# lucanest/Phyloformer

Hardware: AMD Instinct MI355X
Metric: alignments/sec, 60-leaf/500-site LG+GC-like MSAs, Phyloformer forward (pf.ckpt) (higher is better)
Workload: dtype f16x3-split MFMA (two fp16 limbs per operand, 3 passes), fp32 accumulate/residual

## Files before the change

### include/phyloformer_amd.h

```cpp
#ifndef PHYLOFORMER_AMD_H
#define PHYLOFORMER_AMD_H

#include <stddef.h>
#include <stdint.h>

#ifdef __cplusplus
extern "C" {
#endif

#define PF_ABI_VERSION 5

typedef enum pf_status {
    PF_OK = 0,
    PF_EINVAL = -1,
    PF_EHIP = -2,
    PF_ERCCL = -3,
    PF_ENOMEM = -4,
    PF_ESTATE = -5,
    PF_EIO = -6
} pf_status;

typedef struct pf_weights_t {
    int32_t n_blocks;
    int32_t n_heads;
// ... 46 lines not shown

int pf_forward_sharded(pf_handle_t* h, const uint8_t* idx, int32_t B, int32_t N,
                       int32_t l_begin, int32_t l_end, int32_t L_total, float* out);
int pf_forward_sharded_device(pf_handle_t* h, const uint8_t* d_idx, int32_t B, int32_t N,
                              int32_t l_begin, int32_t l_end, int32_t L_total, float* d_out);

#define PF_UNIQUE_ID_BYTES 256
int pf_comm_unique_id(void* id_out);
int pf_comm_init(pf_handle_t* h, const void* unique_id, int32_t rank, int32_t world_size);
int pf_comm_destroy(pf_handle_t* h);
int pf_comm_info(char* path_out, size_t path_cap, int32_t* version);

int pf_synchronize(pf_handle_t* h);
int pf_get_stream(pf_handle_t* h, void** hip_stream_out);
int pf_device_malloc(pf_handle_t* h, size_t bytes, void** out);
int pf_device_free(pf_handle_t* h, void* p);
int pf_memcpy_h2d(pf_handle_t* h, void* dst, const void* src, size_t bytes);
int pf_memcpy_d2h(pf_handle_t* h, void* dst, const void* src, size_t bytes);

int pf_profile_reset(pf_handle_t* h);
int pf_profile_get(pf_handle_t* h, const char* kernel, int64_t* launches, double* total_ms);

int64_t pf_debug_read(pf_handle_t* h, const char* name, float* dst, int64_t cap);

int pf_device_info(pf_handle_t* h, char* name_out, size_t name_cap, int32_t* cu_count,
                   uint64_t* hbm_bytes);
int pf_device_pci(pf_handle_t* h, int32_t* domain, int32_t* bus, int32_t* device);

int pf_forward_shards_emulated(pf_handle_t* h, const uint8_t* idx, int32_t B, int32_t N, int32_t L,
                               int32_t nshards, float* out);

int pf_selftest(pf_handle_t* h, float* out);

typedef struct pf_mha_weights_t {
    int32_t n_heads;
    int32_t embed_dim;
    const float *wq, *bq, *wk, *bk, *wv, *bv, *wo, *bo;
} pf_mha_weights_t;
typedef struct pf_mha pf_mha_t;
int pf_create_bare(int device, pf_handle_t** out);
int pf_mha_create(pf_handle_t* h, const pf_mha_weights_t* w, pf_mha_t** out);
int pf_mha_destroy(pf_mha_t* m);
int pf_mha_forward(pf_mha_t* m, const float* x, int32_t B, int32_t R, int32_t C, float* y);
int pf_mha_forward_device(pf_mha_t* m, const float* d_x, int32_t B, int32_t R, int32_t C, float* d_y);

#define PF_FASTA_EBYTE (-16)
#define PF_FASTA_ERAGGED (-17)
#define PF_FASTA_ENOHEADER (-18)
#define PF_FASTA_EEMPTY (-19)
#define PF_FASTA_ECAP (-20)
#define PF_FASTA_EUTF8 (-21)
int pf_parse_fasta(const char* data, int64_t len, uint8_t* idx, int64_t idx_cap, int64_t* id_spans,
                   int32_t max_seqs, int32_t* n_out, int32_t* l_out, int64_t* detail);

int64_t pf_format_phylip(const float* preds, int32_t n, const char* const* ids, char* out, int64_t cap);
int64_t pf_format_phylip_n(const float* preds, int32_t n, const char* const* ids, const int64_t* id_lens, char* out,
                           int64_t cap);

int64_t pf_nj_newick_n(const float* preds, int32_t n, const char* const* ids, const int64_t* id_lens, int32_t clamp_negative,
                       char* out, int64_t cap);

typedef struct pf_fasta_batch pf_fasta_batch_t;
int pf_fasta_batch_load(const char* const* paths, int32_t count, int32_t threads, pf_fasta_batch_t** out);
void pf_fasta_batch_free(pf_fasta_batch_t* b);
int32_t pf_fasta_batch_count(const pf_fasta_batch_t* b);
int pf_fasta_batch_infos(const pf_fasta_batch_t* b, int32_t* status, int32_t* n, int32_t* l, int64_t* detail);
// ... 12 lines not shown
```

### phyloformer_amd/csrc/pf_device.hip.h

```cpp
#pragma once
#include <hip/hip_runtime.h>
#include <stdint.h>

#include "pf_layout.h"

namespace pfk {

typedef float f32x4 __attribute__((ext_vector_type(4)));
typedef float f32x16 __attribute__((ext_vector_type(16)));
#if PF_F16
typedef _Float16 h16_t;
#define PF_MFMA(a, b, c) __builtin_amdgcn_mfma_f32_32x32x16_f16((a), (b), (c), 0, 0, 0)
#define PF_DOT2C "v_dot2c_f32_f16"
#define PF_CVT_PK "v_cvt_pk_f16_f32"
#define PF_NEG1_LO 0x0000bc00u
#define PF_NEG1_HI 0xbc000000u
#else
typedef __bf16 h16_t;
#define PF_MFMA(a, b, c) __builtin_amdgcn_mfma_f32_32x32x16_bf16((a), (b), (c), 0, 0, 0)
#define PF_DOT2C "v_dot2c_f32_bf16"
#define PF_CVT_PK "v_cvt_pk_bf16_f32"
#define PF_NEG1_LO 0x0000bf80u
#define PF_NEG1_HI 0xbf800000u
#endif
// ... 242 lines not shown
        xn[j] = x[j] - mean;
        v4[j & 3] = fmaf(xn[j], xn[j], v4[j & 3]);
    }
    const float v = (v4[0] + v4[1]) + (v4[2] + v4[3]);
    const float rstd = __builtin_amdgcn_rsqf(pair_sum(v) * (1.f / 64.f) + LN_EPS);
#pragma unroll
    for (int j = 0; j < 32; ++j) xn[j] *= rstd;
}

typedef const f32x4 __attribute__((address_space(3)))* lds_f32x4_t;
__device__ __forceinline__ void load_acc_bias(f32x16& acc, lds_f32_t lds_bias_h) {
#pragma unroll
    for (int q4 = 0; q4 < 4; ++q4) {
        const f32x4 bb = *(lds_f32x4_t)(lds_bias_h + 8 * q4);
#pragma unroll
        for (int i = 0; i < 4; ++i) acc[4 * q4 + i] = bb[i];
    }
}

__device__ __forceinline__ void load_acc_bias(f32x16& acc, const float* lds_bias, int h) {
#pragma unroll
    for (int q4 = 0; q4 < 4; ++q4) {
        const f32x4 bb = *reinterpret_cast<const f32x4*>(lds_bias + 8 * q4 + 4 * h);
#pragma unroll
        for (int i = 0; i < 4; ++i) acc[4 * q4 + i] = bb[i];
    }
}

__device__ __forceinline__ frag_t zero_frag() {
    frag_t z;
#pragma unroll
    for (int i = 0; i < 8; ++i) z[i] = (h16_t)0.f;
    return z;
}

#ifndef PF_DEVICE_HELPERS_ONLY
struct MainArgs {
    float* x;
    float* qrow;
    const float* qcol;
    const frag_t* mfrag;
    const float* rq;
    const float* ctx;
    float* spart;
    float* outpart;
    const frag_t* wimg;
    const float* consts;
    const frag_t* wv_lo;
    const float* table;
    const uint8_t* idx;
    const int16_t* pair_i;
    const int16_t* pair_j;
    int B, N, P, Lloc;
    int flat;
    int nt_aln;
    int slots_aln;
    size_t trash_tok;
    int store_x_last;
    unsigned long long* prof;
    int ablate;
    float* sitemap;
};

enum { MODE_FIRST = 0, MODE_MID = 1, MODE_LAST = 2, MODE_MID0 = 3, MODE_LAST_FOLD = 4 };

struct TilePos { int b, kt, r0, l0; };
// ... 52 lines not shown
    constexpr bool FOLD = MODE == MODE_LAST_FOLD;
    static_assert(!SITEMAP || LAST, "the site map is the head's: last block only");
    extern __shared__ __attribute__((aligned(16))) unsigned char smem[];
    lds_frag_t lw = (lds_frag_t)smem;
    lds_f32_t lc = (lds_f32_t)(smem + FRAG_END * 16);

    {
        const float cv = a.consts[min((int)threadIdx.x, CONST_LEN - 1)];
        if (FOLD) {
            image_to_lds<FRAG_W1, FRAG_W2>(a.wimg, smem);
            image_to_lds<FRAG_WO, FRAG_U + U_FRAGS>(a.wimg, smem);
        } else {
            image_to_lds<(MODE == MODE_FIRST) ? FRAG_WV : 0, LAST ? FRAG_WV : FRAG_END>(a.wimg, smem);
        }
        static_assert(CONST_LEN <= MAIN_THREADS, "one constant per thread");
        if (threadIdx.x < CONST_LEN) reinterpret_cast<float*>(smem + FRAG_END * 16)[threadIdx.x] = cv;
        asm volatile("s_waitcnt vmcnt(0)" ::: "memory");
    }
    __syncthreads();

    const int lane = threadIdx.x & 63;
    const int wave = __builtin_amdgcn_readfirstlane(threadIdx.x >> 6);
    const int t = lane & 31;
    const int h = lane >> 5;
    const int ntiles = (a.Lloc + 31) >> 5;
    const int ntasks = a.B * a.nt_aln;
    if (wave >= MAIN_WAVES / 2) __builtin_amdgcn_s_setprio(1);
    unsigned long long tacc[6] = {0, 0, 0, 0, 0, 0}, tprev = 0;
#define PF_TICK(k) do { if (a.prof) { const unsigned long long tn_ = __builtin_amdgcn_s_memtime(); tacc[k] += tn_ - tprev; tprev = tn_; } } while (0)
    if (a.prof) tprev = __builtin_amdgcn_s_memtime();
    lds_frag_t w1p = lw + FRAG_W1 + lane;
    lds_frag_t w2p = lw + FRAG_W2 + lane;
    lds_frag_t wop = lw + FRAG_WO + lane;
    lds_frag_t qkp = lw + FRAG_QK + h * 8 + (t & 7);
    lds_f32_t lch = lc + 4 * h;
    PF_OPAQUE(wop); PF_OPAQUE(qkp); PF_OPAQUE(lch);
    lds_frag_t wvp = wop + (FRAG_WV - FRAG_WO);
    lds_f32_t luh = (lds_f32_t)(smem + FRAG_U * 16) + 16 * h;

    {
        const int nwaves = gridDim.x * MAIN_WAVES;
#ifndef PF_RUN_MAX
#define PF_RUN_MAX 8
#endif
        const int run = max(1, min(PF_RUN_MAX, ntasks / (nwaves * 8)));
        int run0 = (blockIdx.x * MAIN_WAVES + wave) * run;
        const int task0 = run0, task1 = ntasks;
        TilePos cur = tile_pos<FLAT>(a, min(task0, ntasks - 1), ntiles);
        int frag_row = -1;
        frag_t mfr[4];
        f32x4 rqv = {0.f, 0.f, 0.f, 0.f};
        f32x4 px[8], pctx[8], pqr, pqc;
        int pri = 0, prj = 0;
        auto prefetch = [&](const TilePos& np) {
            const LanePos nl = lane_pos<FLAT>(a, np, t);
            const int ll = nl.l, pb = np.b;
            const size_t tk = nl.tok0 + nl.toff;
            if (MODE == MODE_MID0) {
                const uint8_t* ib = a.idx + (size_t)pb * a.N * a.Lloc + ll;
                const int pp = np.r0 + (nl.in_r1 ? 1 : 0);
                pri = residue(ib[(size_t)a.pair_i[pp] * a.Lloc]);
                prj = residue(ib[(size_t)a.pair_j[pp] * a.Lloc]);
            } else {
                const f32x4* xp = reinterpret_cast<const f32x4*>(a.x + tk * 64 + 4 * h);
#pragma unroll
                for (int g = 0; g < 8; ++g) px[g] = xp[2 * g];
            }
            pqr = *reinterpret_cast<const f32x4*>(a.qrow + tk * 4);
            pqc = *reinterpret_cast<const f32x4*>(a.qcol + tk * 4);
            if (MODE != MODE_FIRST) {
                int hq = h;
                asm volatile("" : "+v"(hq));
                const f32x4* cp = reinterpret_cast<const f32x4*>(a.ctx + ((size_t)pb * a.Lloc + ll) * 64 + 4 * hq);
#pragma unroll
                for (int g = 0; g < 8; ++g) pctx[g] = cp[2 * g];
            }
        };
        if (MODE != MODE_FIRST && task0 < task1) prefetch(cur);

        for (int task = task0; task < task1;) {
            const int b = cur.b;
            const int row = b * a.P + cur.r0;
            int ntask = task + 1;
            TilePos nxt = tile_next<FLAT>(a, cur);
            if (ntask == run0 + run) {
                run0 += nwaves * run;
                ntask = run0;
                if (ntask < task1) nxt = tile_pos<FLAT>(a, ntask, ntiles);
            }
            const LanePos lp = lane_pos<FLAT>(a, cur, t);
            const bool straddle = lp.wrap < 32;
            int ai = 0, aj = 0;
            if (MODE == MODE_FIRST) { const int pp = cur.r0 + (lp.in_r1 ? 1 : 0); ai = a.pair_i[pp]; aj = a.pair_j[pp]; }
            auto load_mfr = [&](int r) {
                const frag_t* mf = a.mfrag + (size_t)r * 128 + t;
#pragma unroll
                for (int q = 0; q < 4; ++q) mfr[q] = mf[q * 32];
                typedef const f32x4 __attribute__((address_space(4)))* const_f32x4_t;
                rqv = *(const_f32x4_t)(unsigned long long)(a.rq + (size_t)__builtin_amdgcn_readfirstlane(r) * 4);
                frag_row = r;
            };
            if (MODE != MODE_FIRST && row != frag_row) load_mfr(row);
            const bool valid = lp.valid;
            const int lc_ = lp.l;
            const size_t tok = lp.tok0 + lp.toff;
            float x[32];
            float zh[4] = {0.f, 0.f, 0.f, 0.f};

            if (MODE == MODE_FIRST) {
                const int ri = residue(a.idx[((size_t)b * a.N + ai) * a.Lloc + lc_]);
                const int rj = residue(a.idx[((size_t)b * a.N + aj) * a.Lloc + lc_]);
                const f32x4* ti = reinterpret_cast<const f32x4*>(a.table + ri * 64 + 4 * h);
                const f32x4* tj = reinterpret_cast<const f32x4*>(a.table + rj * 64 + 4 * h);
#pragma unroll
                for (int g = 0; g < 8; ++g) {
                    f32x4 u = ti[2 * g], w = tj[2 * g];
#pragma unroll
                    for (int i = 0; i < 4; ++i) x[4 * g + i] = u[i] + w[i];
                }
            } else {
                if (MODE == MODE_MID0) {
                    const f32x4* ti = reinterpret_cast<const f32x4*>(a.table + pri * 64 + 4 * h);
                    const f32x4* tj = reinterpret_cast<const f32x4*>(a.table + prj * 64 + 4 * h);
#pragma unroll
                    for (int g = 0; g < 8; ++g) {
                        const f32x4 u = ti[2 * g], w = tj[2 * g];
#pragma unroll
                        for (int i = 0; i < 4; ++i) x[4 * g + i] = u[i] + w[i];
                    }
                } else {
#pragma unroll
                    for (int g = 0; g < 8; ++g)
#pragma unroll
                        for (int i = 0; i < 4; ++i) x[4 * g + i] = px[g][i];
                }
                PF_TICK(0);
                if (!(a.ablate & 8)) {
                    f32x16 ya[2];
#pragma unroll
                    for (int j = 0; j < 32; ++j) ya[j >> 4][j & 15] = x[j];
                    {
                        const f32x4 qr = pqr;
                        auto mix = [&](const bool mine) {
                            float v[8];
#pragma unroll
                            for (int i = 0; i < 4; ++i) v[i] = mine ? qr[i] * rqv[i] : 0.f;
                            v[4] = v[5] = mine ? 1.f : 0.f;
                            v[6] = v[7] = 0.f;
                            frag_t qb_hi, qb_lo;
                            split8(v, qb_hi, qb_lo);
#pragma unroll
                            for (int To = 0; To < 2; ++To) mfma3(ya[To], mfr[To * 2], mfr[To * 2 + 1], qb_hi, qb_lo, To == 1);
                        };
                        mix(h == 0 && !lp.in_r1);
                        if (straddle) {
                            load_mfr(row + 1);
                            mix(h == 0 && lp.in_r1);
                        }
                    }
                    {
                        const f32x4 qc = pqc * COLAPPLY_B_SCALE;
                        float o[32];
#pragma unroll
                        for (int g = 0; g < 8; ++g) {
                            const f32x4 u = pctx[g];
#pragma unroll
                            for (int i = 0; i < 4; ++i) o[4 * g + i] = u[i] * qc[g >> 1];
                        }
#pragma unroll
                        for (int s = 0; s < 4; ++s) {
                            frag_t ob_hi, ob_lo;
                            split8(&o[8 * s], ob_hi, ob_lo);
#pragma unroll
                            for (int To = 0; To < 2; ++To) {
                                lds_frag_t f = wop + ((To * 4 + s) * 2) * 64;
                                const frag_t a_hi = f[0], a_lo = f[64];
                                mfma3(ya[To], a_hi, a_lo, ob_hi, ob_lo, To == 1);
                            }
                        }
                    }
#pragma unroll
                    for (int j = 0; j < 32; ++j) x[j] = ya[j >> 4][j & 15];
                }

                PF_TICK(1);
                if (FOLD) {
#pragma unroll
                    for (int g = 0; g < 8; ++g) {
                        const f32x4 w4 = *(lds_f32x4_t)(lch + CONST_HW + 8 * g);
#pragma unroll
// ... 80 lines not shown
                            }
                            mfma3(oa[To], fh, fl, g_hi[u], g_lo[u], To == 1);
                            fh = nh; fl = nl;
                        }
                    }
                    PF_TICK(3);
#pragma unroll
                    for (int j = 0; j < 32; ++j) x[j] = oa[j >> 4][j & 15];
                }
            }

            if (!LAST && !(a.ablate & 4)) {
                frag_t wl[8];
#pragma unroll
                for (int i = WVLO_LDS; i < 8; ++i) wl[i] = a.wv_lo[i * 64 + lane];
                __builtin_amdgcn_sched_barrier(0);
                {
                    const size_t stok = valid ? tok : a.trash_tok + t;
                    f32x4* xo = reinterpret_cast<f32x4*>(a.x + stok * 64 + 4 * h);
#pragma unroll
                    for (int g = 0; g < 8; ++g) {
                        f32x4 u = {x[4 * g], x[4 * g + 1], x[4 * g + 2], x[4 * g + 3]};
                        xo[2 * g] = u;
                    }
                }
                if (a.ablate & 32) { cur = nxt; task = ntask; continue; }
                f32x16 va[3];
                {
                    float xn[32];
                    ln_pair(x, xn);
                    frag_t xb_hi[4], xb_lo[4];
#pragma unroll
                    for (int s = 0; s < 4; ++s) split8(&xn[8 * s], xb_hi[s], xb_lo[s]);
#pragma unroll
                    for (int s = 0; s < 4; ++s) {
                        const frag_t q_hi = qkp[(s * 2) * 16], q_lo = qkp[(s * 2 + 1) * 16];
                        if (s == 0) mfma3_zero(va[2], q_hi, q_lo, xb_hi[s], xb_lo[s]);
                        else mfma3(va[2], q_hi, q_lo, xb_hi[s], xb_lo[s]);
                    }
#pragma unroll
                    for (int s = 0; s < 4; ++s)
#pragma unroll
                        for (int T = 0; T < 2; ++T) {
                            const frag_t f_hi = wvp[(T * 4 + s) * 64];
                            const frag_t f_lo = T * 4 + s < WVLO_LDS ? wvp[(FRAG_WVLO - FRAG_WV) + (T * 4 + s) * 64] : wl[T * 4 + s];
                            if (s == 0) mfma3_zero(va[T], f_hi, f_lo, xb_hi[s], xb_lo[s], T == 1);
                            else mfma3(va[T], f_hi, f_lo, xb_hi[s], xb_lo[s], T == 1);
                        }
                }
#pragma unroll
                for (int r = 0; r < 4; ++r) va[2][r] += lc[CONST_BQK + 4 * h + r];
                float qk[4], ot[4];
#pragma unroll
                for (int i = 0; i < 4; ++i) qk[i] = elu1_fast(va[2][i]);
#pragma unroll
                for (int i = 0; i < 4; ++i) ot[i] = pair_other(qk[i], h);
                float qn[4], kn[4];
#pragma unroll
                for (int i = 0; i < 4; ++i) {
                    qn[i] = h ? ot[i] : qk[i];
                    kn[i] = h ? qk[i] : ot[i];
                }
                {
                    const size_t stok = valid ? tok : a.trash_tok + t;
                    f32x4 qs = {qn[0], qn[1], qn[2], qn[3]};
                    *reinterpret_cast<f32x4*>(a.qrow + stok * 4) = qs;
                }
                const long slot0 = (long)b * a.slots_aln + cur.kt + (FLAT ? cur.r0 : 0);
                for (int part = 0; part < (straddle ? 2 : 1); ++part) {
                    float* sp = a.spart + (size_t)(slot0 + part) * SROW;
                    const float vm = (valid && lp.in_r1 == (part == 1)) ? 1.f : 0.f;
                    float km[4];
// ... 214 lines not shown
    }
    __syncthreads();
    if (ok) {
        const float* s = st[sub];
        const int hh = c >> 4;
        const float sk = s[68 + hh];
        ctx[sub][c] = (s[c] + bvc * sk) / sk;
        if (c < 4) {
            const float r = a.L_total / s[64 + c];
            rqs[sub][c] = r;
            a.rq[(size_t)pr * 4 + c] = r * a.b_scale;
        }
    }
    __syncthreads();
    if (ok) {
        float* m = a.mrow ? a.mrow + (size_t)pr * MROW : nullptr;
#pragma unroll
        for (int hh = 0; hh < 4; ++hh) {
            float acc = 0.f;
#pragma unroll
            for (int d = 0; d < 16; ++d) acc = fmaf(wo[hh][d], ctx[sub][16 * hh + d], acc);
            if (m) m[hh * 64 + c] = acc * rqs[sub][hh];
            mm[sub][hh][c] = acc * a.a_scale;
        }
        mm[sub][4][c] = biasc;
        mm[sub][5][c] = biascol;
    }
    __syncthreads();
    if (ok) {
        const int To = c >> 5, t = c & 31;
        float v[8];
#pragma unroll
        for (int i = 0; i < 8; ++i) v[i] = (i < 6) ? mm[sub][i][32 * To + t] : 0.f;
        frag_t hi, lo;
        split8(v, hi, lo);
        frag_t* mf = a.mfrag + (size_t)pr * MFRAG_PER_PAIR + To * 64 + t;
        mf[0] = hi;
        mf[32] = lo;
    }
    }
}

__global__ void k_rowsum(const float* spart, float* srow, int npairs, int nparts_, int flat, int P, int Lloc, int slots_aln) {
    const int i = blockIdx.x * blockDim.x + threadIdx.x;
    if (i >= npairs * SROW) return;
    const int pr = i / SROW, c = i - pr * SROW;
    long first;
    int nparts;
    part_range(flat, pr, nparts_, P, Lloc, slots_aln, &first, &nparts);
    const float* sp = spart + (size_t)first * SROW + c;
    float acc = 0.f;
    for (int k = 0; k < nparts; k += 8) {
        float v[8];
#pragma unroll
        for (int q = 0; q < 8; ++q) v[q] = k + q < nparts ? sp[(size_t)(k + q) * SROW] : 0.f;
#pragma unroll
        for (int q = 0; q < 8; ++q) acc += v[q];
    }
    srow[i] = acc;
}

__global__ void k_outsum(const float* outpart, float* out, int npairs, int nparts_, float inv_L_total, int flat, int P,
                         int Lloc, int slots_aln) {
    const int pr = blockIdx.x * blockDim.x + threadIdx.x;
    if (pr >= npairs) return;
    long first;
    int nparts;
    part_range(flat, pr, nparts_, P, Lloc, slots_aln, &first, &nparts);
    const float* sp = outpart + first;
    float acc = 0.f;
    for (int k = 0; k < nparts; k += 8) {
// ... 394 lines not shown

__global__ void k_accumulate(float* dst, const float* src, size_t n) {
    const size_t i = (size_t)blockIdx.x * blockDim.x + threadIdx.x;
    if (i < n) dst[i] += src[i];
}

__global__ void k_selftest(float* out) {
    const int lane = threadIdx.x;
    out[lane] = pair_sum((float)lane);
    out[64 + lane] = pair_other((float)lane, lane >> 5);
    out[128 + lane] = row16_sum((float)lane);
    out[192 + lane] = half32_sum((float)lane);
    frag_t A1, A2, Bf;
    const int m = lane & 31, kg = lane >> 5;
#pragma unroll
    for (int i = 0; i < 8; ++i) {
        const int k = 8 * kg + i;
        A1[i] = (h16_t)(float)(m + 32 * (k % 8));
        A2[i] = (h16_t)(float)k;
        Bf[i] = (h16_t)((k == (m & 15)) ? 1.f : 0.f);
    }
    f32x16 acc1, acc2;
#pragma unroll
    for (int r = 0; r < 16; ++r) { acc1[r] = 0.f; acc2[r] = 0.f; }
    acc1 = PF_MFMA(A1, Bf, acc1);
    acc2 = PF_MFMA(A2, Bf, acc2);
#pragma unroll
    for (int r = 0; r < 16; ++r) {
        out[256 + lane * 16 + r] = acc1[r];
        out[1280 + lane * 16 + r] = acc2[r];
    }
}

#endif

}
```

### phyloformer_amd/csrc/pf_host_prep.h

```cpp
#pragma once
#include <algorithm>
#include <cmath>
#include <cstdint>
#include <cstring>
#include <vector>

#include "pf_layout.h"

namespace pfhost {
using namespace pfk;

inline uint16_t f2bf(float f) {
    uint32_t u;
    std::memcpy(&u, &f, 4);
    if ((u & 0x7fffffffu) > 0x7f800000u) return uint16_t((u >> 16) | 0x40);
    u += 0x7fffu + ((u >> 16) & 1u);
    return uint16_t(u >> 16);
}
inline float bf2f(uint16_t b) {
    uint32_t u = uint32_t(b) << 16;
    float f;
    std::memcpy(&f, &u, 4);
    return f;
}
// ... 31 lines not shown
#if PF_F16
inline uint16_t f2x(float f) { return f2h(f); }
inline float x2f(uint16_t b) { return h2f(b); }
#else
inline uint16_t f2x(float f) { return f2bf(f); }
inline float x2f(uint16_t b) { return bf2f(b); }
#endif
inline int kmap_h(int j, int h) { return 8 * (j >> 2) + 4 * h + (j & 3); }

inline void pack_frags(const float* W, int M, int K, int Mpad, uint16_t* out, float scale = 1.f) {
    const int nT = Mpad / 32, nS = K / 16;
    for (int T = 0; T < nT; ++T)
        for (int s = 0; s < nS; ++s)
            for (int lane = 0; lane < 64; ++lane)
                for (int i = 0; i < 8; ++i) {
                    const int m = 32 * T + (lane & 31), k = kmap_h(8 * s + i, lane >> 5);
                    const float w = (m < M) ? W[(size_t)m * K + k] * scale : 0.f;
                    const uint16_t hi = f2x(w);
                    const uint16_t lo = f2x(w - x2f(hi));
                    const size_t base = ((size_t)(T * nS + s) * 2) * 64;
                    out[(base + lane) * 8 + i] = hi;
                    out[(base + 64 + lane) * 8 + i] = lo;
                }
}

inline void pack_qk_frags(const float* wq, const float* wk, uint16_t* qk) {
    for (int s = 0; s < 4; ++s)
        for (int kg = 0; kg < 2; ++kg)
            for (int m = 0; m < 8; ++m)
                for (int i = 0; i < 8; ++i) {
                    const int k = kmap_h(8 * s + i, kg);
                    const float w = (m < 4) ? wq[(size_t)m * E + k] : wk[(size_t)(m - 4) * E + k];
                    const uint16_t hi = f2x(w), lo = f2x(w - x2f(hi));
                    qk[(((size_t)s * 2 + 0) * 16 + kg * 8 + m) * 8 + i] = hi;
                    qk[(((size_t)s * 2 + 1) * 16 + kg * 8 + m) * 8 + i] = lo;
                }
}

inline void pack_row_stats(const float* wv, const float* wq, const float* wk, uint16_t* img_tail ,
                    uint16_t* wv_lo) {
    std::vector<uint16_t> full((size_t)2 * 4 * 2 * 64 * 8);
    pack_frags(wv, E, E, E, full.data());
    for (int T = 0; T < 2; ++T)
        for (int s = 0; s < 4; ++s)
            for (int lane = 0; lane < 64; ++lane)
                for (int i = 0; i < 8; ++i) {
                    const size_t src = (((size_t)(T * 4 + s) * 2) * 64 + lane) * 8 + i;
                    const size_t dst = ((size_t)(T * 4 + s) * 64 + lane) * 8 + i;
                    img_tail[dst] = full[src];
                    wv_lo[dst] = full[src + 64 * 8];
                }
    pack_qk_frags(wq, wk, img_tail + (size_t)(FRAG_QK - FRAG_WV) * 8);
}

inline void fold_head(const float* w2 , const float* b2, const float* hw, float hb, double w2_scale,
                      float* u_img , float* c0) {
    for (int T = 0; T < FF / 32; ++T)
        for (int h = 0; h < 2; ++h)
            for (int r = 0; r < 16; ++r) {
                const int k = 32 * T + kmap_h(r, h);
                double acc = 0.0;
                for (int c = 0; c < E; ++c) acc += (double)hw[c] * (double)w2[(size_t)c * FF + k];
                u_img[(T * 2 + h) * 16 + r] = (float)(acc * w2_scale);
            }
    double acc = (double)hb;
    for (int c = 0; c < E; ++c) acc += (double)hw[c] * (double)b2[c];
    *c0 = (float)acc;
}

// ... 132 lines not shown
```

### phyloformer_amd/csrc/pf_layout.h

```cpp
#pragma once

#ifndef PF_F16
#define PF_F16 1
#endif

namespace pfk {

constexpr int E = 64;
constexpr int NH = 4;
constexpr int HD = 16;
constexpr int FF = 256;
constexpr int NA = 22;
constexpr int SROW = 72;
constexpr int MROW = 4 * 64;
constexpr float LN_EPS = 1e-5f;

constexpr int FRAG_W1 = 0;
constexpr int FRAG_W2 = FRAG_W1 + 8 * 4 * 2 * 64;
constexpr int FRAG_WO = FRAG_W2 + 2 * 16 * 2 * 64;
constexpr int FRAG_WV = FRAG_WO + 2 * 4 * 2 * 64;
constexpr int FRAG_QK = FRAG_WV + 2 * 4 * 64;
#ifndef PF_WVLO_LDS
#define PF_WVLO_LDS 4
#endif
constexpr int WVLO_LDS = PF_WVLO_LDS;
constexpr int FRAG_WVLO = FRAG_QK + 4 * 2 * 16;
constexpr int FRAG_END = FRAG_WVLO + WVLO_LDS * 64;
constexpr int FRAG_U = FRAG_WV;
constexpr int U_FRAGS = FF * 4 / 16;
static_assert(FRAG_U + U_FRAGS <= FRAG_END, "the folded head fits the last block's tail");
constexpr int WVLO_FRAGS = 2 * 4 * 64;
constexpr int CONST_B1 = 0, CONST_B2 = 256, CONST_BQK = 320, CONST_HW = 328, CONST_HB = 392,
              CONST_C0 = 393, CONST_BOC = 400;
constexpr int CONST_LEN = 464;
constexpr int MAIN_LDS_BYTES = FRAG_END * 16 + CONST_LEN * 4;
constexpr int MFRAG_PER_PAIR = 2 * 2 * 32;

constexpr int MAIN_THREADS = 512;
constexpr int MAIN_WAVES = MAIN_THREADS / 64;

constexpr int PAIRTAB_ROWS = 22 * 22, PAIRTAB_W = 72;

}
```

### phyloformer_amd/csrc/pf_lib.hip

```cpp
#include <hip/hip_runtime.h>
#include <dlfcn.h>

#include <algorithm>
#include <cmath>
#include <cstdarg>
#include <cstdio>
#include <cstdlib>
#include <cstring>
#include <functional>
#include <map>
#include <mutex>
#include <string>
#include <vector>

#include "../../include/phyloformer_amd.h"
#include "pf_device.hip.h"
#include "pf_mha.hip.h"
#include "pf_precise.hip.h"
#include "pf_generic.hip.h"
#include "pf_boot.hip.h"
#include "pf_sites.hip.h"
#include "pf_sitemap.hip.h"
#include "pf_sites_host.h"
#include "pf_host_prep.h"
// ... 1701 lines not shown
    float* total = (float*)stage.alloc((size_t)B * P * SROW * sizeof(float));
    if (!total) return fail(h, PF_ENOMEM, "shard sum buffer");
    auto reduce = [&](bool site_sums) -> int {
        const size_t count = (size_t)B * P * (site_sums ? 1 : SROW);
        for (ShardRun& r : runs)
            if (!site_sums && (rc = launch_rowsum(h, r, &r.rs))) return rc;
        hipMemsetAsync(total, 0, count * sizeof(float), h->stream);
        for (ShardRun& r : runs) {
            hipLaunchKernelGGL(k_accumulate, dim3((unsigned)((count + 255) / 256)), dim3(256), 0, h->stream,
                               total, site_sums ? r.d_out : r.w.srow, count);
            r.rs = RowStats{total, 1, 0};
        }
        return PF_OK;
    };
    rc = schedule(h, runs.data(), runs.size(), reduce);
    if (!rc && (hipMemcpyAsync(out, total, (size_t)B * P * sizeof(float), hipMemcpyDeviceToHost, h->stream) != hipSuccess ||
                hipStreamSynchronize(h->stream) != hipSuccess))
        rc = fail(h, PF_EHIP, "result copy failed");
    return rc;
}

int pf_selftest(pf_handle_t* h, float* out) {
    if (!h || !out) return PF_EINVAL;
    float* d = nullptr;
    HIPCHK(h, hipMalloc((void**)&d, 2304 * sizeof(float)));
    hipLaunchKernelGGL(k_selftest, dim3(1), dim3(64), 0, h->stream, d);
    HIPCHK(h, hipGetLastError());
    HIPCHK(h, hipMemcpyAsync(out, d, 2304 * sizeof(float), hipMemcpyDeviceToHost, h->stream));
    HIPCHK(h, hipStreamSynchronize(h->stream));
    hipFree(d);
    return PF_OK;
}

struct pf_mha {
    pf_handle* h = nullptr;
    float* wfrag = nullptr;
    float* bias = nullptr;
    char* ws = nullptr;
    size_t ws_bytes = 0;
    float* d_x = nullptr;
    float* d_y = nullptr;
    size_t d_xy_bytes = 0;
};

int pf_mha_create(pf_handle_t* h, const pf_mha_weights_t* w, pf_mha_t** out) {
    if (!h || !w || !out) return PF_EINVAL;
    if (w->n_heads != MHA_H || w->embed_dim != E)
        return fail(h, PF_EINVAL, "softmax attention kernels are specialised for embed_dim 64 / 4 heads, got %d / %d",
                    w->embed_dim, w->n_heads);
    const float* ws[4] = {w->wq, w->wk, w->wv, w->wo};
    const float* bs[4] = {w->bq, w->bk, w->bv, w->bo};
    std::vector<uint16_t> img((size_t)MHA_WTOTAL * 8);
    std::vector<float> bias(4 * E);
    for (int i = 0; i < 4; ++i) {
        if (!ws[i] || !bs[i]) return fail(h, PF_EINVAL, "pf_mha_create: NULL weight pointer");
        std::copy(bs[i], bs[i] + E, bias.begin() + i * E);
    }
    pack_frags(w->wq, E, E, E, img.data());
    pack_frags(w->wk, E, E, E, img.data() + (size_t)MHA_OFF_WK * 8);
    pack_frags(w->wv, E, E, E, img.data() + (size_t)MHA_OFF_WV * 8);
    pack_frags(w->wo, E, E, E, img.data() + (size_t)MHA_OFF_WO * 8);
    HIPCHK(h, hipSetDevice(h->device));
    pf_mha* m = new pf_mha();
    m->h = h;
    void* p = nullptr;
    if (hipMalloc(&p, img.size() * 2) != hipSuccess) { delete m; return fail(h, PF_ENOMEM, "pf_mha_create: hipMalloc failed"); }
// ... 101 lines not shown
```

### phyloformer_amd/engine.py

```python
from __future__ import annotations

import ctypes as C
import os
from typing import Dict, Optional, Tuple

import numpy as np

from .weights import ModelWeights

HERE = os.path.dirname(os.path.abspath(__file__))
LIB_PATH = os.path.join(HERE, "libphyloformer_amd.so")
ABI_VERSION = 5
UNIQUE_ID_BYTES = 256

PF_OK, PF_EINVAL, PF_EHIP, PF_ERCCL, PF_ENOMEM, PF_ESTATE = 0, -1, -2, -3, -4, -5


def _refuse_single_sequence(B: int, N: int):
    if N == 1 and B >= 1:
        raise RuntimeError(f"cannot reshape tensor of 0 elements into shape [{B}, -1, 0, 64] because the unspecified "
                           "dimension size -1 can be any value and is ambiguous")


class EngineError(RuntimeError):
# ... 21 lines not shown
    "pf_forward_device": (C.c_int, [_H, C.c_void_p, C.c_int32, C.c_int32, C.c_int32, C.c_void_p]),
    "pf_resample_sites_device": (C.c_int, [_H, C.c_void_p, C.c_int32, C.c_int32, C.c_int32, C.c_int32, C.c_int32,
                                           C.c_uint64, C.c_void_p]),
    "pf_bootstrap": (C.c_int, [_H, C.c_void_p, C.c_int32, C.c_int32, C.c_int32, C.c_int32, C.c_uint64, C.c_void_p]),
    "pf_window_count": (C.c_int, [C.c_int32, C.c_int32, C.c_int32]),
    "pf_window_start": (C.c_int, [C.c_int32, C.c_int32, C.c_int32, C.c_int32]),
    "pf_gather_sites_device": (C.c_int, [_H, C.c_void_p, C.c_int32, C.c_int32, C.c_int32, C.c_void_p, C.c_void_p,
                                         C.c_int32, C.c_int32, C.c_void_p]),
    "pf_forward_sites": (C.c_int, [_H, C.c_void_p, C.c_int32, C.c_int32, C.c_int32, C.c_void_p, C.c_int32, C.c_int32,
                                   C.c_void_p]),
    "pf_forward_windows": (C.c_int, [_H, C.c_void_p, C.c_int32, C.c_int32, C.c_int32, C.c_int32, C.c_int32, C.c_void_p,
                                     C.c_int32]),
    "pf_forward_sharded": (C.c_int, [_H, C.c_void_p, C.c_int32, C.c_int32, C.c_int32, C.c_int32,
                                     C.c_int32, C.c_void_p]),
    "pf_forward_sharded_device": (C.c_int, [_H, C.c_void_p, C.c_int32, C.c_int32, C.c_int32,
                                            C.c_int32, C.c_int32, C.c_void_p]),
    "pf_comm_unique_id": (C.c_int, [C.c_void_p]),
    "pf_comm_init": (C.c_int, [_H, C.c_void_p, C.c_int32, C.c_int32]),
    "pf_comm_destroy": (C.c_int, [_H]),
    "pf_comm_info": (C.c_int, [C.c_char_p, C.c_size_t, C.POINTER(C.c_int32)]),
    "pf_synchronize": (C.c_int, [_H]),
    "pf_get_stream": (C.c_int, [_H, C.POINTER(C.c_void_p)]),
    "pf_device_malloc": (C.c_int, [_H, C.c_size_t, C.POINTER(C.c_void_p)]),
    "pf_device_free": (C.c_int, [_H, C.c_void_p]),
    "pf_memcpy_h2d": (C.c_int, [_H, C.c_void_p, C.c_void_p, C.c_size_t]),
    "pf_memcpy_d2h": (C.c_int, [_H, C.c_void_p, C.c_void_p, C.c_size_t]),
    "pf_profile_reset": (C.c_int, [_H]),
    "pf_profile_get": (C.c_int, [_H, C.c_char_p, C.POINTER(C.c_int64), C.POINTER(C.c_double)]),
    "pf_debug_read": (C.c_int64, [_H, C.c_char_p, C.c_void_p, C.c_int64]),
    "pf_device_info": (C.c_int, [_H, C.c_char_p, C.c_size_t, C.POINTER(C.c_int32),
                                 C.POINTER(C.c_uint64)]),
    "pf_device_pci": (C.c_int, [_H, C.POINTER(C.c_int32), C.POINTER(C.c_int32), C.POINTER(C.c_int32)]),
    "pf_selftest": (C.c_int, [_H, C.c_void_p]),
    "pf_create_bare": (C.c_int, [C.c_int, C.POINTER(_H)]),
    "pf_mha_create": (C.c_int, [_H, C.c_void_p, C.POINTER(C.c_void_p)]),
    "pf_mha_destroy": (C.c_int, [C.c_void_p]),
    "pf_mha_forward": (C.c_int, [C.c_void_p, C.c_void_p, C.c_int32, C.c_int32, C.c_int32, C.c_void_p]),
    "pf_mha_forward_device": (C.c_int, [C.c_void_p, C.c_void_p, C.c_int32, C.c_int32, C.c_int32, C.c_void_p]),
    "pf_parse_fasta": (C.c_int, [C.c_char_p, C.c_int64, C.c_void_p, C.c_int64, C.c_void_p, C.c_int32,
                                 C.POINTER(C.c_int32), C.POINTER(C.c_int32), C.POINTER(C.c_int64)]),
    "pf_format_phylip": (C.c_int64, [C.c_void_p, C.c_int32, C.POINTER(C.c_char_p), C.c_char_p, C.c_int64]),
    "pf_format_phylip_n": (C.c_int64, [C.c_void_p, C.c_int32, C.POINTER(C.c_char_p), C.c_void_p, C.c_char_p, C.c_int64]),
    "pf_fasta_batch_load": (C.c_int, [C.POINTER(C.c_char_p), C.c_int32, C.c_int32, C.POINTER(C.c_void_p)]),
    "pf_fasta_batch_free": (None, [C.c_void_p]),
    "pf_fasta_batch_count": (C.c_int32, [C.c_void_p]),
    "pf_fasta_batch_infos": (C.c_int, [C.c_void_p, C.c_void_p, C.c_void_p, C.c_void_p, C.c_void_p]),
    "pf_fasta_batch_id": (C.c_int, [C.c_void_p, C.c_int32, C.c_int32, C.POINTER(C.c_void_p), C.POINTER(C.c_int64)]),
    "pf_fasta_batch_gather": (C.c_int, [C.c_void_p, C.c_void_p, C.c_int32, C.c_int32, C.c_int32, C.c_void_p]),
    "pf_nj_newick_n": (C.c_int64, [C.c_void_p, C.c_int32, C.POINTER(C.c_char_p), C.c_void_p, C.c_int32, C.c_char_p, C.c_int64]),
    "pf_phylip_write_batch": (C.c_int, [C.c_void_p, C.c_void_p, C.c_int32, C.c_int32, C.c_void_p,
                                        C.POINTER(C.c_char_p), C.POINTER(C.c_char_p), C.c_int32, C.c_void_p]),
    "pf_forward_shards_emulated": (C.c_int, [_H, C.c_void_p, C.c_int32, C.c_int32, C.c_int32, C.c_int32,
                                             C.c_void_p]),
    "pf_forward_site_map": (C.c_int, [_H, C.c_void_p, C.c_int32, C.c_int32, C.c_int32, C.c_void_p, C.c_void_p]),
    "pf_forward_site_map_device": (C.c_int, [_H, C.c_void_p, C.c_int32, C.c_int32, C.c_int32, C.c_void_p, C.c_void_p]),
    "pf_forward_site_profile": (C.c_int, [_H, C.c_void_p, C.c_int32, C.c_int32, C.c_int32, C.c_void_p, C.c_void_p,
                                          C.c_void_p]),
    "pf_site_moments_device": (C.c_int, [_H, C.c_void_p, C.c_int32, C.c_int32, C.c_int32, C.c_void_p, C.c_void_p]),
}

CALL_TIME_SYMBOLS = frozenset({"pf_forward_site_map", "pf_forward_site_map_device", "pf_forward_site_profile",
                               "pf_site_moments_device"})

_lib: Optional[C.CDLL] = None


# ... 281 lines not shown
    def collective_count(self) -> int:
        return self.profile_get("collectives")[0]

    def rechecked_count(self) -> int:
        return self.profile_get("rechecked")[0]

    def comm_info(self) -> dict:
        buf = C.create_string_buffer(512)
        ver = C.c_int32()
        rc = self._lib.pf_comm_info(buf, 512, C.byref(ver))
        if rc != PF_OK:
            raise EngineError(rc, (self._lib.pf_last_error(None) or b"").decode())
        return {"library": buf.value.decode(), "version": int(ver.value)}

    def profile_reset(self):
        self._check(self._lib.pf_profile_reset(self._h))

    def profile_get(self, kernel: str) -> Tuple[int, float]:
        n = C.c_int64()
        ms = C.c_double()
        self._check(self._lib.pf_profile_get(self._h, kernel.encode(), C.byref(n), C.byref(ms)))
        return n.value, ms.value

    def debug_read(self, name: str) -> np.ndarray:
        n = self._check(self._lib.pf_debug_read(self._h, name.encode(), None, 0))
        out = np.empty(n, dtype=np.float32)
        self._check(self._lib.pf_debug_read(self._h, name.encode(), out.ctypes.data, n))
        return out

    def selftest(self) -> np.ndarray:
        out = np.empty(2304, dtype=np.float32)
        self._check(self._lib.pf_selftest(self._h, out.ctypes.data))
        return out
```

Measured before the change: 527.0.

## Stack hi/lo fp16 limbs into single MFMA K-dimension for mix and QK projections

New measurement: 531.8, median of 6. About the same (+0.9%).

```diff
diff --git a/include/phyloformer_amd.h b/include/phyloformer_amd.h
--- a/include/phyloformer_amd.h
+++ b/include/phyloformer_amd.h
@@ -102,6 +102,8 @@
 
 int pf_selftest(pf_handle_t* h, float* out);
 
+int pf_selftest_stacked(pf_handle_t* h, float* out);
+
 typedef struct pf_mha_weights_t {
     int32_t n_heads;
     int32_t embed_dim;
diff --git a/phyloformer_amd/csrc/pf_device.hip.h b/phyloformer_amd/csrc/pf_device.hip.h
--- a/phyloformer_amd/csrc/pf_device.hip.h
+++ b/phyloformer_amd/csrc/pf_device.hip.h
@@ -298,6 +298,26 @@
 #pragma unroll
     for (int i = 0; i < 8; ++i) z[i] = (h16_t)0.f;
     return z;
+}
+
+__device__ __forceinline__ void stack_mix_frags(const frag_t& hi, const frag_t& lo, frag_t& f0, frag_t& f1) {
+#pragma unroll
+    for (int i = 0; i < 6; ++i) f0[i] = hi[i];
+    f0[6] = lo[0]; f0[7] = lo[1];
+#pragma unroll
+    for (int i = 0; i < 4; ++i) { f1[i] = lo[2 + i]; f1[4 + i] = hi[i]; }
+}
+__device__ __forceinline__ frag_t mix_b_frag(unsigned qh0, unsigned ql0, unsigned qh1, unsigned ql1, unsigned one, int h) {
+    u32x4 b;
+    b[0] = h ? qh1 : qh0;
+    b[1] = h ? one : qh1;
+    b[2] = h ? ql0 : one;
+    b[3] = h ? ql1 : qh0;
+    return __builtin_bit_cast(frag_t, b);
+}
+__device__ __forceinline__ unsigned packed_ones() {
+    const h16x2 o = {(h16_t)1.f, (h16_t)1.f};
+    return __builtin_bit_cast(unsigned, o);
 }
 
 #ifndef PF_DEVICE_HELPERS_ONLY
@@ -416,7 +436,7 @@
     lds_frag_t w1p = lw + FRAG_W1 + lane;
     lds_frag_t w2p = lw + FRAG_W2 + lane;
     lds_frag_t wop = lw + FRAG_WO + lane;
-    lds_frag_t qkp = lw + FRAG_QK + h * 8 + (t & 7);
+    lds_frag_t qkp = lw + FRAG_QK + h * 16 + (t & 15);
     lds_f32_t lch = lc + 4 * h;
     PF_OPAQUE(wop); PF_OPAQUE(qkp); PF_OPAQUE(lch);
     lds_frag_t wvp = wop + (FRAG_WV - FRAG_WO);
@@ -432,7 +452,7 @@
         const int task0 = run0, task1 = ntasks;
         TilePos cur = tile_pos<FLAT>(a, min(task0, ntasks - 1), ntiles);
         int frag_row = -1;
-        frag_t mfr[4];
+        frag_t mfr[2];
         f32x4 rqv = {0.f, 0.f, 0.f, 0.f};
         f32x4 px[8], pctx[8], pqr, pqc;
         int pri = 0, prj = 0;
@@ -477,9 +497,9 @@
             int ai = 0, aj = 0;
             if (MODE == MODE_FIRST) { const int pp = cur.r0 + (lp.in_r1 ? 1 : 0); ai = a.pair_i[pp]; aj = a.pair_j[pp]; }
             auto load_mfr = [&](int r) {
-                const frag_t* mf = a.mfrag + (size_t)r * 128 + t;
-#pragma unroll
-                for (int q = 0; q < 4; ++q) mfr[q] = mf[q * 32];
+                const frag_t* mf = a.mfrag + (size_t)r * MFRAG_PER_PAIR + lane;
+#pragma unroll
+                for (int To = 0; To < 2; ++To) mfr[To] = mf[To * 64];
                 typedef const f32x4 __attribute__((address_space(4)))* const_f32x4_t;
                 rqv = *(const_f32x4_t)(unsigned long long)(a.rq + (size_t)__builtin_amdgcn_readfirstlane(r) * 4);
                 frag_row = r;
@@ -526,20 +546,20 @@
                     {
                         const f32x4 qr = pqr;
                         auto mix = [&](const bool mine) {
-                            float v[8];
+                            float v[4];
 #pragma unroll
                             for (int i = 0; i < 4; ++i) v[i] = mine ? qr[i] * rqv[i] : 0.f;
-                            v[4] = v[5] = mine ? 1.f : 0.f;
-                            v[6] = v[7] = 0.f;
-                            frag_t qb_hi, qb_lo;
-                            split8(v, qb_hi, qb_lo);
-#pragma unroll
-                            for (int To = 0; To < 2; ++To) mfma3(ya[To], mfr[To * 2], mfr[To * 2 + 1], qb_hi, qb_lo, To == 1);
+                            unsigned qh0, ql0, qh1, ql1;
+                            split_pair(v[0], v[1], qh0, ql0);
+                            split_pair(v[2], v[3], qh1, ql1);
+                            const frag_t qb = mix_b_frag(qh0, ql0, qh1, ql1, mine ? packed_ones() : 0u, h);
+#pragma unroll
+                            for (int To = 0; To < 2; ++To) ya[To] = PF_MFMA(mfr[To], qb, ya[To]);
                         };
-                        mix(h == 0 && !lp.in_r1);
+                        mix(!lp.in_r1);
                         if (straddle) {
                             load_mfr(row + 1);
-                            mix(h == 0 && lp.in_r1);
+                            mix(lp.in_r1);
                         }
                     }
                     {
@@ -686,12 +706,16 @@
                     frag_t xb_hi[4], xb_lo[4];
 #pragma unroll
                     for (int s = 0; s < 4; ++s) split8(&xn[8 * s], xb_hi[s], xb_lo[s]);
+                    f32x16 vl;
+                    const f32x16 z = {0.f, 0.f, 0.f, 0.f, 0.f, 0.f, 0.f, 0.f, 0.f, 0.f, 0.f, 0.f, 0.f, 0.f, 0.f, 0.f};
 #pragma unroll
                     for (int s = 0; s < 4; ++s) {
-                        const frag_t q_hi = qkp[(s * 2) * 16], q_lo = qkp[(s * 2 + 1) * 16];
-                        if (s == 0) mfma3_zero(va[2], q_hi, q_lo, xb_hi[s], xb_lo[s]);
-                        else mfma3(va[2], q_hi, q_lo, xb_hi[s], xb_lo[s]);
+                        const frag_t qf = qkp[s * 32];
+                        vl = PF_MFMA(qf, xb_lo[s], s == 0 ? z : vl);
+                        va[2] = PF_MFMA(qf, xb_hi[s], s == 0 ? z : va[2]);
                     }
+#pragma unroll
+                    for (int r = 0; r < 4; ++r) va[2][r] = (vl[r] + va[2][r]) + va[2][4 + r];
 #pragma unroll
                     for (int s = 0; s < 4; ++s)
 #pragma unroll
@@ -972,11 +996,12 @@
         float v[8];
 #pragma unroll
         for (int i = 0; i < 8; ++i) v[i] = (i < 6) ? mm[sub][i][32 * To + t] : 0.f;
-        frag_t hi, lo;
+        frag_t hi, lo, f0, f1;
         split8(v, hi, lo);
+        stack_mix_frags(hi, lo, f0, f1);
         frag_t* mf = a.mfrag + (size_t)pr * MFRAG_PER_PAIR + To * 64 + t;
-        mf[0] = hi;
-        mf[32] = lo;
+        mf[0] = f0;
+        mf[32] = f1;
     }
     }
 }
@@ -1437,6 +1462,46 @@
     }
 }
 
+__global__ void k_selftest_stacked(float* out) {
+    const int lane = threadIdx.x, t = lane & 31, h = lane >> 5;
+    f32x16 z;
+#pragma unroll
+    for (int r = 0; r < 16; ++r) z[r] = 0.f;
+    {
+        frag_t hi = zero_frag(), lo = zero_frag(), f0, f1;
+#pragma unroll
+        for (int j = 0; j < 6; ++j) {
+            hi[j] = (h16_t)(float)((7 * t + 13 * j) % 31 + 1);
+            lo[j] = (h16_t)(float)((5 * t + 11 * j) % 29 + 1);
+        }
+        stack_mix_frags(hi, lo, f0, f1);
+        h16x2 qh[2], ql[2];
+#pragma unroll
+        for (int i = 0; i < 4; ++i) {
+            qh[i >> 1][i & 1] = (h16_t)(float)((3 * t + 17 * i) % 23 + 1);
+            ql[i >> 1][i & 1] = (h16_t)(float)((9 * t + 5 * i) % 19 + 1);
+        }
+        const frag_t b = mix_b_frag(__builtin_bit_cast(unsigned, qh[0]), __builtin_bit_cast(unsigned, ql[0]),
+                                    __builtin_bit_cast(unsigned, qh[1]), __builtin_bit_cast(unsigned, ql[1]), packed_ones(), h);
+        const f32x16 d = PF_MFMA(h ? f1 : f0, b, z);
+#pragma unroll
+        for (int r = 0; r < 16; ++r) out[lane * 16 + r] = d[r];
+    }
+    {
+        frag_t af, bf;
+        const int row = t & 15;
+#pragma unroll
+        for (int i = 0; i < 8; ++i) {
+            const int k = 8 * h + i;
+            af[i] = (h16_t)(float)(row < 8 ? (7 * row + 3 * k) % 17 + 1 : (11 * (row - 8) + 5 * k) % 13 + 1);
+            bf[i] = (h16_t)(float)((5 * k + 3 * t) % 11 + 1);
+        }
+        const f32x16 d = PF_MFMA(af, bf, z);
+#pragma unroll
+        for (int e = 0; e < 8; ++e) out[1024 + lane * 8 + e] = d[e];
+    }
+}
+
 #endif
 
 }
diff --git a/phyloformer_amd/csrc/pf_host_prep.h b/phyloformer_amd/csrc/pf_host_prep.h
--- a/phyloformer_amd/csrc/pf_host_prep.h
+++ b/phyloformer_amd/csrc/pf_host_prep.h
@@ -87,9 +87,20 @@
                     const int k = kmap_h(8 * s + i, kg);
                     const float w = (m < 4) ? wq[(size_t)m * E + k] : wk[(size_t)(m - 4) * E + k];
                     const uint16_t hi = f2x(w), lo = f2x(w - x2f(hi));
-                    qk[(((size_t)s * 2 + 0) * 16 + kg * 8 + m) * 8 + i] = hi;
-                    qk[(((size_t)s * 2 + 1) * 16 + kg * 8 + m) * 8 + i] = lo;
-                }
+                    qk[(((size_t)s * 2 + kg) * 16 + 0 + m) * 8 + i] = hi;
+                    qk[(((size_t)s * 2 + kg) * 16 + 8 + m) * 8 + i] = lo;
+                }
+}
+
+inline void stack_mix_frags(const uint16_t hi[6], const uint16_t lo[6], uint16_t f0[8], uint16_t f1[8]) {
+    for (int i = 0; i < 6; ++i) f0[i] = hi[i];
+    f0[6] = lo[0]; f0[7] = lo[1];
+    for (int i = 0; i < 4; ++i) { f1[i] = lo[2 + i]; f1[4 + i] = hi[i]; }
+}
+inline void mix_b_frag(const uint16_t qh[4], const uint16_t ql[4], uint16_t one, int h, uint16_t b[8]) {
+    const uint16_t h0[8] = {qh[0], qh[1], qh[2], qh[3], one, one, qh[0], qh[1]};
+    const uint16_t h1[8] = {qh[2], qh[3], one, one, ql[0], ql[1], ql[2], ql[3]};
+    for (int i = 0; i < 8; ++i) b[i] = h ? h1[i] : h0[i];
 }
 
 inline void pack_row_stats(const float* wv, const float* wq, const float* wk, uint16_t* img_tail ,
diff --git a/phyloformer_amd/csrc/pf_layout.h b/phyloformer_amd/csrc/pf_layout.h
--- a/phyloformer_amd/csrc/pf_layout.h
+++ b/phyloformer_amd/csrc/pf_layout.h
@@ -34,7 +34,7 @@
               CONST_C0 = 393, CONST_BOC = 400;
 constexpr int CONST_LEN = 464;
 constexpr int MAIN_LDS_BYTES = FRAG_END * 16 + CONST_LEN * 4;
-constexpr int MFRAG_PER_PAIR = 2 * 2 * 32;
+constexpr int MFRAG_PER_PAIR = 2 * 64;
 
 constexpr int MAIN_THREADS = 512;
 constexpr int MAIN_WAVES = MAIN_THREADS / 64;
diff --git a/phyloformer_amd/csrc/pf_lib.hip b/phyloformer_amd/csrc/pf_lib.hip
--- a/phyloformer_amd/csrc/pf_lib.hip
+++ b/phyloformer_amd/csrc/pf_lib.hip
@@ -1757,6 +1757,18 @@
     return PF_OK;
 }
 
+int pf_selftest_stacked(pf_handle_t* h, float* out) {
+    if (!h || !out) return PF_EINVAL;
+    float* d = nullptr;
+    HIPCHK(h, hipMalloc((void**)&d, 1536 * sizeof(float)));
+    hipLaunchKernelGGL(k_selftest_stacked, dim3(1), dim3(64), 0, h->stream, d);
+    HIPCHK(h, hipGetLastError());
+    HIPCHK(h, hipMemcpyAsync(out, d, 1536 * sizeof(float), hipMemcpyDeviceToHost, h->stream));
+    HIPCHK(h, hipStreamSynchronize(h->stream));
+    hipFree(d);
+    return PF_OK;
+}
+
 struct pf_mha {
     pf_handle* h = nullptr;
     float* wfrag = nullptr;
diff --git a/phyloformer_amd/engine.py b/phyloformer_amd/engine.py
--- a/phyloformer_amd/engine.py
+++ b/phyloformer_amd/engine.py
@@ -77,6 +77,7 @@
                                  C.POINTER(C.c_uint64)]),
     "pf_device_pci": (C.c_int, [_H, C.POINTER(C.c_int32), C.POINTER(C.c_int32), C.POINTER(C.c_int32)]),
     "pf_selftest": (C.c_int, [_H, C.c_void_p]),
+    "pf_selftest_stacked": (C.c_int, [_H, C.c_void_p]),
     "pf_create_bare": (C.c_int, [C.c_int, C.POINTER(_H)]),
     "pf_mha_create": (C.c_int, [_H, C.c_void_p, C.POINTER(C.c_void_p)]),
     "pf_mha_destroy": (C.c_int, [C.c_void_p]),
@@ -424,3 +425,8 @@
         out = np.empty(2304, dtype=np.float32)
         self._check(self._lib.pf_selftest(self._h, out.ctypes.data))
         return out
+
+    def selftest_stacked(self) -> np.ndarray:
+        out = np.empty(1536, dtype=np.float32)
+        self._check(self._lib.pf_selftest_stacked(self._h, out.ctypes.data))
+        return out
```
